# rpng/open_vins

Hardware: NVIDIA H100
Metric: msckf_updates_per_sec (higher is better)
Workload: dtype f64

## Files before the change

open_vins_b200/csrc/k_triangulate.cu:

```cuda
#include "geom.cuh"

__global__ void k_cam_poses(const DevFrame *fr, DevCamPoses *cc) {
  OVB_PDL_ENTER();
  int idx = blockIdx.x * blockDim.x + threadIdx.x;
  int total = fr->n_cams * fr->n_clones;
  if (idx >= total)
    return;
  int cam = idx / fr->n_clones, cl = idx % fr->n_clones;
  dm3 R_ItoC = ld_m3(fr->cam_R[cam]);
  dv3 p_IinC = ld_v3(fr->cam_p[cam]);
  dm3 R_GtoI = ld_m3(fr->clone_R[cl]);
  dv3 p_IinG = ld_v3(fr->clone_p[cl]);
  dm3 R = mul33(R_ItoC, R_GtoI);
  dv3 p = sub3(p_IinG, mTv3(R, p_IinC));
#pragma unroll
  for (int i = 0; i < 9; i++)
    cc->cc_R[cam][cl][i] = R.m[i];
  cc->cc_p[cam][cl][0] = p.x;
  cc->cc_p[cam][cl][1] = p.y;
  cc->cc_p[cam][cl][2] = p.z;
}

void launch_cam_poses(ovb_ctx *ctx) {
  int total = OVB_MAX_CAMS * OVB_MAX_CLONES;
  k_cam_poses<<<(total + 127) / 128, 128, 0, ctx->stream>>>(ctx->d_frame, ctx->d_cc);
}

#define TRI_MAX_WARPS 8
#define TRI_PITCH 33
template <int NV> __device__ __forceinline__ void seq_add(double (&s)[NV], const double (&c)[NV], int count, double *wbuf) {
  const int lane = threadIdx.x & 31;
#pragma unroll
  for (int k = 0; k < NV; k++)
    wbuf[k * TRI_PITCH + lane] = c[k];
  __syncwarp();
  double a = 0.0;
#pragma unroll
  for (int k = 0; k < NV; k++)
    a = (lane == k) ? s[k] : a;
  if (lane < NV) {
    const double *row = wbuf + lane * TRI_PITCH;
    for (int l = 0; l < count; l++)
      a += row[l];
  }
#pragma unroll
  for (int k = 0; k < NV; k++)
    s[k] = __shfl_sync(0xffffffffu, a, k);
  __syncwarp();
}

struct Rel {
  dm3 R;
  dv3 t;
  dv3 q;
};
__device__ __forceinline__ Rel rel_pose(const DevCamPoses *fr, int cam, int cl, const dm3 &R_GtoA, dv3 p_AinG) {
  dm3 Rc = ld_m3(fr->cc_R[cam][cl]);
  dv3 pc = ld_v3(fr->cc_p[cam][cl]);
  Rel r;
  r.R = mul33T(Rc, R_GtoA);
  r.t = mv3(R_GtoA, sub3(pc, p_AinG));
  r.q = negmv3(r.R, r.t);
  return r;
}

__device__ __forceinline__ double lm_cost(const DevCamPoses *fr, const BlobView &bv, int m0, int m1, int lane, const dm3 &R_GtoA, dv3 p_AinG,
                                          double alpha, double beta, double rho, double *wbuf) {
  double err[1] = {0.0};
  for (int base = m0; base < m1; base += 32) {
    const int i = base + lane;
    double c[1] = {0.0};
    if (i < m1) {
      Rel r = rel_pose(fr, bv.cam[i], bv.clone[i], R_GtoA, p_AinG);
      double hi1 = r.R.m[0] * alpha + r.R.m[1] * beta + r.R.m[2] + rho * r.q.x;
      double hi2 = r.R.m[3] * alpha + r.R.m[4] * beta + r.R.m[5] + rho * r.q.y;
      double hi3 = r.R.m[6] * alpha + r.R.m[7] * beta + r.R.m[8] + rho * r.q.z;
      float z0 = (float)(hi1 / hi3), z1 = (float)(hi2 / hi3);
      float r0 = __fsub_rn(bv.uvn[2 * i], z0), r1 = __fsub_rn(bv.uvn[2 * i + 1], z1);
      float nrm = __fsqrt_rn(__fadd_rn(__fmul_rn(r0, r0), __fmul_rn(r1, r1)));
      c[0] = (double)nrm * (double)nrm;
    }
    seq_add<1>(err, c, min(32, m1 - base), wbuf);
  }
  return err[0];
}

__global__ void __launch_bounds__(256) k_triangulate(const DevCamPoses *__restrict__ fr, const DevOpts *__restrict__ dop,
                                                     DevFeat *__restrict__ feats, int n_feats, BlobView bv) {
  OVB_PDL_ENTER();
  __shared__ double tri_stage[TRI_MAX_WARPS][9 * TRI_PITCH];
  double *wbuf = tri_stage[threadIdx.x >> 5];
  int warp = (blockIdx.x * blockDim.x + threadIdx.x) >> 5;
  int lane = threadIdx.x & 31;
  if (warp >= n_feats)
    return;
  DevFeat *F = &feats[warp];
  const ovb_opts &op = dop->o;
  int m0 = F->m0, m1 = F->m1;
  const double qnan = __longlong_as_double(0x7ff8000000000000LL);
  int status = OVB_FEAT_OK;
  dv3 pA = mk3(qnan, qnan, qnan), pG = pA;
  int anchor_cam = -1, anchor_clone = -1;
  if (m1 - m0 < 2) {
    status = OVB_FEAT_FEW_MEAS;
  } else {
    int most = 0;
    anchor_cam = 0;
    for (int k = F->key0; k < F->key1; k++) {
      int key = bv.keys[k];
      int cnt = 0;
      for (int i = m0 + lane; i < m1; i += 32)
        cnt += (bv.cam[i] == key) ? 1 : 0;
#pragma unroll
      for (int o = 16; o > 0; o >>= 1)
        cnt += __shfl_xor_sync(0xffffffffu, cnt, o);
      if (cnt > most) {
        anchor_cam = key;
        most = cnt;
      }
    }
    int ameas = -1;
    for (int i = m0 + lane; i < m1; i += 32)
      if (bv.cam[i] == anchor_cam)
        ameas = i;
#pragma unroll
    for (int o = 16; o > 0; o >>= 1)
      ameas = max(ameas, __shfl_xor_sync(0xffffffffu, ameas, o));
    anchor_clone = bv.clone[ameas];
    dm3 R_GtoA = ld_m3(fr->cc_R[anchor_cam][anchor_clone]);
    dv3 p_AinG = ld_v3(fr->cc_p[anchor_cam][anchor_clone]);
    dv3 p_f;
    if (!op.triangulate_1d) {
      double Ab[9] = {0, 0, 0, 0, 0, 0, 0, 0, 0};
      for (int base = m0; base < m1; base += 32) {
        const int i = base + lane;
        double c[9] = {0, 0, 0, 0, 0, 0, 0, 0, 0};
        if (i < m1) {
          Rel r = rel_pose(fr, bv.cam[i], bv.clone[i], R_GtoA, p_AinG);
          dv3 bi = mTv3(r.R, mk3((double)bv.uvn[2 * i], (double)bv.uvn[2 * i + 1], 1.0));
          double nb = norm3(bi);
          bi = mk3(bi.x / nb, bi.y / nb, bi.z / nb);
          dm3 Bp = skew3(bi);
          dm3 Ai = mulT33(Bp, Bp);
          dv3 Aip = mv3(Ai, r.t);
          c[0] = Ai.m[0], c[1] = Ai.m[1], c[2] = Ai.m[2], c[3] = Ai.m[4], c[4] = Ai.m[5], c[5] = Ai.m[8];
          c[6] = Aip.x, c[7] = Aip.y, c[8] = Aip.z;
        }
        seq_add<9>(Ab, c, min(32, m1 - base), wbuf);
      }
      double A[9] = {Ab[0], Ab[1], Ab[2], Ab[1], Ab[3], Ab[4], Ab[2], Ab[4], Ab[5]};
      double b[3] = {Ab[6], Ab[7], Ab[8]};
      p_f = colpiv_solve3(A, mk3(b[0], b[1], b[2]));
      double condA = cond_sym3(A);
      if (fabs(condA) > op.max_cond_number)
        status = OVB_FEAT_TRI_COND;
      else if (p_f.z < op.min_dist || p_f.z > op.max_dist)
        status = OVB_FEAT_TRI_DEPTH;
      else if (isnan(norm3(p_f)))
        status = OVB_FEAT_TRI_NAN;
    } else {
      dv3 ba = mk3((double)bv.uvn[2 * ameas], (double)bv.uvn[2 * ameas + 1], 1.0);
      double nba = norm3(ba);
      ba = mk3(ba.x / nba, ba.y / nba, ba.z / nba);
      double Ab1[2] = {0.0, 0.0};
      for (int base = m0; base < m1; base += 32) {
        const int i = base + lane;
        double c[2] = {0.0, 0.0};
        if (i < m1 && i != ameas) {
          Rel r = rel_pose(fr, bv.cam[i], bv.clone[i], R_GtoA, p_AinG);
          dv3 bi = mTv3(r.R, mk3((double)bv.uvn[2 * i], (double)bv.uvn[2 * i + 1], 1.0));
          double nb = norm3(bi);
          bi = mk3(bi.x / nb, bi.y / nb, bi.z / nb);
          dm3 Bp = skew3(bi);
          dv3 Bb = mv3(Bp, ba);
          c[0] = dot3(Bb, Bb);
          c[1] = dot3(Bb, mv3(Bp, r.t));
        }
        seq_add<2>(Ab1, c, min(32, m1 - base), wbuf);
      }
      const double A1 = Ab1[0], b1 = Ab1[1];
      double depth = b1 / A1;
      p_f = mk3(depth * ba.x, depth * ba.y, depth * ba.z);
      if (p_f.z < op.min_dist || p_f.z > op.max_dist)
        status = OVB_FEAT_TRI_DEPTH;
      else if (isnan(norm3(p_f)))
        status = OVB_FEAT_TRI_NAN;
    }
    if (status == OVB_FEAT_OK) {
      pA = p_f;
      pG = add3(mTv3(R_GtoA, pA), p_AinG);
    }
    if (status == OVB_FEAT_OK && op.refine_features) {
      double rho = 1 / pA.z;
      double alpha = pA.x / pA.z;
      double beta = pA.y / pA.z;
      double lam = op.init_lamda;
      double eps = 10000;
      int runs = 0;
      bool recompute = true;
      double Hs[6] = {0, 0, 0, 0, 0, 0};
      double g[3] = {0, 0, 0};
      double cost_old = lm_cost(fr, bv, m0, m1, lane, R_GtoA, p_AinG, alpha, beta, rho, wbuf);
      while (runs < op.max_runs && lam < op.max_lamda && eps > op.min_dx) {
        if (recompute) {
#pragma unroll
          for (int k = 0; k < 6; k++)
            Hs[k] = 0.0;
          g[0] = g[1] = g[2] = 0.0;
          double Hg[9] = {0, 0, 0, 0, 0, 0, 0, 0, 0};
          for (int base = m0; base < m1; base += 32) {
            const int i = base + lane;
            double c[9] = {0, 0, 0, 0, 0, 0, 0, 0, 0};
            if (i < m1) {
              Rel r = rel_pose(fr, bv.cam[i], bv.clone[i], R_GtoA, p_AinG);
              double hi1 = r.R.m[0] * alpha + r.R.m[1] * beta + r.R.m[2] + rho * r.q.x;
              double hi2 = r.R.m[3] * alpha + r.R.m[4] * beta + r.R.m[5] + rho * r.q.y;
              double hi3 = r.R.m[6] * alpha + r.R.m[7] * beta + r.R.m[8] + rho * r.q.z;
              double h3sq = hi3 * hi3;
              double H0[3], H1[3];
              H0[0] = (r.R.m[0] * hi3 - hi1 * r.R.m[6]) / h3sq;
              H0[1] = (r.R.m[1] * hi3 - hi1 * r.R.m[7]) / h3sq;
              H0[2] = (r.q.x * hi3 - hi1 * r.q.z) / h3sq;
              H1[0] = (r.R.m[3] * hi3 - hi2 * r.R.m[6]) / h3sq;
              H1[1] = (r.R.m[4] * hi3 - hi2 * r.R.m[7]) / h3sq;
              H1[2] = (r.q.y * hi3 - hi2 * r.q.z) / h3sq;
              float z0 = (float)(hi1 / hi3), z1 = (float)(hi2 / hi3);
              double rd0 = (double)__fsub_rn(bv.uvn[2 * i], z0), rd1 = (double)__fsub_rn(bv.uvn[2 * i + 1], z1);
              c[0] = H0[0] * H0[0] + H1[0] * H1[0];
              c[1] = H0[0] * H0[1] + H1[0] * H1[1];
              c[2] = H0[0] * H0[2] + H1[0] * H1[2];
              c[3] = H0[1] * H0[1] + H1[1] * H1[1];
              c[4] = H0[1] * H0[2] + H1[1] * H1[2];
              c[5] = H0[2] * H0[2] + H1[2] * H1[2];
#pragma unroll
              for (int a = 0; a < 3; a++)
                c[6 + a] = H0[a] * rd0 + H1[a] * rd1;
            }
            seq_add<9>(Hg, c, min(32, m1 - base), wbuf);
          }
#pragma unroll
          for (int k = 0; k < 6; k++)
            Hs[k] = Hg[k];
#pragma unroll
          for (int k = 0; k < 3; k++)
            g[k] = Hg[6 + k];
        }
        double Hl[9] = {Hs[0] * (1.0 + lam), Hs[1], Hs[2], Hs[1], Hs[3] * (1.0 + lam), Hs[4], Hs[2], Hs[4], Hs[5] * (1.0 + lam)};
        dv3 dx = colpiv_solve3(Hl, mk3(g[0], g[1], g[2]));
        double cost = lm_cost(fr, bv, m0, m1, lane, R_GtoA, p_AinG, alpha + dx.x, beta + dx.y, rho + dx.z, wbuf);
        if (cost <= cost_old && (cost_old - cost) / cost_old < op.min_dcost) {
          alpha += dx.x;
          beta += dx.y;
          rho += dx.z;
          eps = 0;
          break;
        }
        if (cost <= cost_old) {
          recompute = true;
          cost_old = cost;
          alpha += dx.x;
          beta += dx.y;
          rho += dx.z;
          runs++;
          lam = lam / op.lam_mult;
          eps = norm3(dx);
        } else {
          recompute = false;
          lam = lam * op.lam_mult;
        }
      }
      pA = mk3(alpha / rho, beta / rho, 1 / rho);
      dv3 q1, q2;
      householder_tangent3(pA, q1, q2);
      double base_line_max = 0.0;
      for (int i = m0 + lane; i < m1; i += 32) {
        dv3 pc = ld_v3(fr->cc_p[bv.cam[i]][bv.clone[i]]);
        dv3 t = mv3(R_GtoA, sub3(pc, p_AinG));
        double a0 = dot3(q1, t), a1 = dot3(q2, t);
        double bl = sqrt(a0 * a0 + a1 * a1);
        if (bl > base_line_max)
          base_line_max = bl;
      }
      base_line_max = warp_max(base_line_max);
      if (pA.z < op.min_dist || pA.z > op.max_dist)
        status = OVB_FEAT_GN_DEPTH;
      else if ((norm3(pA) / base_line_max) > op.max_baseline)
        status = OVB_FEAT_GN_BASELINE;
      else if (isnan(norm3(pA)))
        status = OVB_FEAT_GN_NAN;
      else
        pG = add3(mTv3(R_GtoA, pA), p_AinG);
    }
  }
  if (lane == 0) {
    F->status = status;
    F->anchor_cam = anchor_cam;
    F->anchor_clone = anchor_clone;
    F->p_FinA[0] = pA.x;
    F->p_FinA[1] = pA.y;
    F->p_FinA[2] = pA.z;
    F->p_FinG[0] = pG.x;
    F->p_FinG[1] = pG.y;
    F->p_FinG[2] = pG.z;
    F->chi2 = qnan;
  }
}

void launch_triangulate(ovb_ctx *ctx, int n_feats, BlobView bv) {
  if (n_feats <= 0)
    return;
  int warps_per_cta = (n_feats + ctx->sm_count - 1) / ctx->sm_count;
  warps_per_cta = warps_per_cta < 1 ? 1 : (warps_per_cta > 8 ? 8 : warps_per_cta);
  int grid = (n_feats + warps_per_cta - 1) / warps_per_cta;
  ovb_launch(ctx, k_triangulate, dim3(grid), dim3(warps_per_cta * 32), (size_t)(0), ctx->d_cc, ctx->d_opts, ctx->d_feat, n_feats, bv);
}
```

Before: 2308.

## Assign one CTA per feature with shared-memory pose cache and parallel LM damping candidates

Triangulation now runs one CTA per feature instead of one warp per feature. Relative poses and measurements are cached in dynamic shared memory, so each LM pass reads them there rather than recomputing them from global memory. When a CTA has several warps, each warp evaluates the LM step with a different damping factor and also computes the Hessian at its candidate point, so rejected steps cost fewer serial rounds. The cost is extra syncthreads, more shared memory per block, a host-side occupancy query that picks the warp count, and an optional clock-based probe path behind an ifdef.

```diff
diff --git a/open_vins_b200/csrc/k_triangulate.cu b/open_vins_b200/csrc/k_triangulate.cu
--- a/open_vins_b200/csrc/k_triangulate.cu
+++ b/open_vins_b200/csrc/k_triangulate.cu
@@ -1,4 +1,6 @@
 #include "geom.cuh"
+
+#include <cstdio>
 
 __global__ void k_cam_poses(const DevFrame *fr, DevCamPoses *cc) {
   OVB_PDL_ENTER();
@@ -26,8 +28,13 @@
   k_cam_poses<<<(total + 127) / 128, 128, 0, ctx->stream>>>(ctx->d_frame, ctx->d_cc);
 }
 
-#define TRI_MAX_WARPS 8
+#ifndef TRI_MAX_WARPS
+#define TRI_MAX_WARPS 4
+#endif
 #define TRI_PITCH 33
+#define TRI_NV 10
+#define TRI_CAND 13
+#define TRI_REL 15
 template <int NV> __device__ __forceinline__ void seq_add(double (&s)[NV], const double (&c)[NV], int count, double *wbuf) {
   const int lane = threadIdx.x & 31;
 #pragma unroll
@@ -48,6 +55,11 @@
     s[k] = __shfl_sync(0xffffffffu, a, k);
   __syncwarp();
 }
+
+__host__ __device__ constexpr size_t tri_smem_bytes(int max_meas, int n_warps) {
+  return sizeof(double) * ((size_t)TRI_REL * max_meas + (size_t)n_warps * (TRI_NV * TRI_PITCH + TRI_CAND)) + sizeof(float) * 2 * (size_t)max_meas;
+}
+static_assert(tri_smem_bytes(OVB_MAX_MEAS_PER_FEAT, TRI_MAX_WARPS) <= 227 * 1024, "the longest track must fit one CTA's shared memory");
 
 struct Rel {
   dm3 R;
@@ -63,131 +75,238 @@
   r.q = negmv3(r.R, r.t);
   return r;
 }
-
-__device__ __forceinline__ double lm_cost(const DevCamPoses *fr, const BlobView &bv, int m0, int m1, int lane, const dm3 &R_GtoA, dv3 p_AinG,
-                                          double alpha, double beta, double rho, double *wbuf) {
-  double err[1] = {0.0};
-  for (int base = m0; base < m1; base += 32) {
-    const int i = base + lane;
-    double c[1] = {0.0};
-    if (i < m1) {
-      Rel r = rel_pose(fr, bv.cam[i], bv.clone[i], R_GtoA, p_AinG);
+__device__ __forceinline__ void rel_store(double *rel, int M, int j, const Rel &r) {
+#pragma unroll
+  for (int k = 0; k < 9; k++)
+    rel[k * M + j] = r.R.m[k];
+  rel[9 * M + j] = r.t.x, rel[10 * M + j] = r.t.y, rel[11 * M + j] = r.t.z;
+  rel[12 * M + j] = r.q.x, rel[13 * M + j] = r.q.y, rel[14 * M + j] = r.q.z;
+}
+__device__ __forceinline__ Rel rel_load(const double *rel, int M, int j) {
+  Rel r;
+#pragma unroll
+  for (int k = 0; k < 9; k++)
+    r.R.m[k] = rel[k * M + j];
+  r.t = mk3(rel[9 * M + j], rel[10 * M + j], rel[11 * M + j]);
+  r.q = mk3(rel[12 * M + j], rel[13 * M + j], rel[14 * M + j]);
+  return r;
+}
+
+template <bool HESS>
+__device__ __forceinline__ void lm_pass(const double *rel, const float *uvn, int M, int lane, double alpha, double beta, double rho,
+                                        double (&s)[TRI_NV], double *wbuf) {
+  constexpr int NV = HESS ? TRI_NV : 1;
+  double a[NV];
+#pragma unroll
+  for (int k = 0; k < NV; k++)
+    a[k] = 0.0;
+  for (int base = 0; base < M; base += 32) {
+    const int j = base + lane;
+    double c[NV];
+#pragma unroll
+    for (int k = 0; k < NV; k++)
+      c[k] = 0.0;
+    if (j < M) {
+      const Rel r = rel_load(rel, M, j);
       double hi1 = r.R.m[0] * alpha + r.R.m[1] * beta + r.R.m[2] + rho * r.q.x;
       double hi2 = r.R.m[3] * alpha + r.R.m[4] * beta + r.R.m[5] + rho * r.q.y;
       double hi3 = r.R.m[6] * alpha + r.R.m[7] * beta + r.R.m[8] + rho * r.q.z;
       float z0 = (float)(hi1 / hi3), z1 = (float)(hi2 / hi3);
-      float r0 = __fsub_rn(bv.uvn[2 * i], z0), r1 = __fsub_rn(bv.uvn[2 * i + 1], z1);
+      float r0 = __fsub_rn(uvn[2 * j], z0), r1 = __fsub_rn(uvn[2 * j + 1], z1);
       float nrm = __fsqrt_rn(__fadd_rn(__fmul_rn(r0, r0), __fmul_rn(r1, r1)));
       c[0] = (double)nrm * (double)nrm;
-    }
-    seq_add<1>(err, c, min(32, m1 - base), wbuf);
-  }
-  return err[0];
-}
-
-__global__ void __launch_bounds__(256) k_triangulate(const DevCamPoses *__restrict__ fr, const DevOpts *__restrict__ dop,
-                                                     DevFeat *__restrict__ feats, int n_feats, BlobView bv) {
+      if constexpr (HESS) {
+        double h3sq = hi3 * hi3;
+        double H0[3], H1[3];
+        H0[0] = (r.R.m[0] * hi3 - hi1 * r.R.m[6]) / h3sq;
+        H0[1] = (r.R.m[1] * hi3 - hi1 * r.R.m[7]) / h3sq;
+        H0[2] = (r.q.x * hi3 - hi1 * r.q.z) / h3sq;
+        H1[0] = (r.R.m[3] * hi3 - hi2 * r.R.m[6]) / h3sq;
+        H1[1] = (r.R.m[4] * hi3 - hi2 * r.R.m[7]) / h3sq;
+        H1[2] = (r.q.y * hi3 - hi2 * r.q.z) / h3sq;
+        double rd0 = (double)r0, rd1 = (double)r1;
+        c[1] = H0[0] * H0[0] + H1[0] * H1[0];
+        c[2] = H0[0] * H0[1] + H1[0] * H1[1];
+        c[3] = H0[0] * H0[2] + H1[0] * H1[2];
+        c[4] = H0[1] * H0[1] + H1[1] * H1[1];
+        c[5] = H0[1] * H0[2] + H1[1] * H1[2];
+        c[6] = H0[2] * H0[2] + H1[2] * H1[2];
+#pragma unroll
+        for (int k = 0; k < 3; k++)
+          c[7 + k] = H0[k] * rd0 + H1[k] * rd1;
+      }
+    }
+    seq_add<NV>(a, c, min(32, M - base), wbuf);
+  }
+#pragma unroll
+  for (int k = 0; k < NV; k++)
+    s[k] = a[k];
+}
+
+__global__ void __launch_bounds__(TRI_MAX_WARPS * 32, 16 / TRI_MAX_WARPS) k_triangulate(const DevCamPoses *__restrict__ fr, const DevOpts *__restrict__ dop,
+                                                                    DevFeat *__restrict__ feats, BlobView bv, int max_meas) {
   OVB_PDL_ENTER();
-  __shared__ double tri_stage[TRI_MAX_WARPS][9 * TRI_PITCH];
-  double *wbuf = tri_stage[threadIdx.x >> 5];
-  int warp = (blockIdx.x * blockDim.x + threadIdx.x) >> 5;
-  int lane = threadIdx.x & 31;
-  if (warp >= n_feats)
-    return;
-  DevFeat *F = &feats[warp];
+#ifdef TRI_PROBE
+  const long long t_start = clock64();
+  long long ts[7] = {0, 0, 0, 0, 0, 0, 0};
+#define TRI_STAMP(k) (ts[k] = clock64())
+  __shared__ int s_passes;
+  int n_acc = 0, n_rej = 0, n_rounds = 0;
+  if (threadIdx.x == 0)
+    s_passes = 0;
+#else
+#define TRI_STAMP(k) ((void)0)
+#endif
+  extern __shared__ double tri_smem[];
+  __shared__ int s_anchor[2];
+  __shared__ int s_status;
+  __shared__ double s_pf[3];
+  __shared__ double s_A[9];
+  __shared__ int s_cond_fail;
+  const int nw = blockDim.x >> 5, warp = threadIdx.x >> 5, lane = threadIdx.x & 31;
+  double *rel = tri_smem;
+  double *wbuf = rel + (size_t)TRI_REL * max_meas + warp * (TRI_NV * TRI_PITCH);
+  double *cand = rel + (size_t)TRI_REL * max_meas + nw * (TRI_NV * TRI_PITCH);
+  float *uvn = (float *)(cand + nw * TRI_CAND);
+  DevFeat *F = &feats[blockIdx.x];
   const ovb_opts &op = dop->o;
-  int m0 = F->m0, m1 = F->m1;
+  const int m0 = F->m0, m1 = F->m1, M = m1 - m0;
   const double qnan = __longlong_as_double(0x7ff8000000000000LL);
   int status = OVB_FEAT_OK;
   dv3 pA = mk3(qnan, qnan, qnan), pG = pA;
   int anchor_cam = -1, anchor_clone = -1;
-  if (m1 - m0 < 2) {
+  if (M < 2) {
     status = OVB_FEAT_FEW_MEAS;
   } else {
-    int most = 0;
-    anchor_cam = 0;
-    for (int k = F->key0; k < F->key1; k++) {
-      int key = bv.keys[k];
-      int cnt = 0;
+    if (warp == 0) {
+      int most = 0;
+      int acam = 0;
+      for (int k = F->key0; k < F->key1; k++) {
+        int key = bv.keys[k];
+        int cnt = 0;
+        for (int i = m0 + lane; i < m1; i += 32)
+          cnt += (bv.cam[i] == key) ? 1 : 0;
+#pragma unroll
+        for (int o = 16; o > 0; o >>= 1)
+          cnt += __shfl_xor_sync(0xffffffffu, cnt, o);
+        if (cnt > most) {
+          acam = key;
+          most = cnt;
+        }
+      }
+      int ameas = -1;
       for (int i = m0 + lane; i < m1; i += 32)
-        cnt += (bv.cam[i] == key) ? 1 : 0;
+        if (bv.cam[i] == acam)
+          ameas = i;
 #pragma unroll
       for (int o = 16; o > 0; o >>= 1)
-        cnt += __shfl_xor_sync(0xffffffffu, cnt, o);
-      if (cnt > most) {
-        anchor_cam = key;
-        most = cnt;
-      }
-    }
-    int ameas = -1;
-    for (int i = m0 + lane; i < m1; i += 32)
-      if (bv.cam[i] == anchor_cam)
-        ameas = i;
-#pragma unroll
-    for (int o = 16; o > 0; o >>= 1)
-      ameas = max(ameas, __shfl_xor_sync(0xffffffffu, ameas, o));
+        ameas = max(ameas, __shfl_xor_sync(0xffffffffu, ameas, o));
+      if (lane == 0)
+        s_anchor[0] = acam, s_anchor[1] = ameas;
+    }
+    __syncthreads();
+    TRI_STAMP(0);
+    anchor_cam = s_anchor[0];
+    const int ameas = s_anchor[1];
     anchor_clone = bv.clone[ameas];
     dm3 R_GtoA = ld_m3(fr->cc_R[anchor_cam][anchor_clone]);
     dv3 p_AinG = ld_v3(fr->cc_p[anchor_cam][anchor_clone]);
-    dv3 p_f;
-    if (!op.triangulate_1d) {
-      double Ab[9] = {0, 0, 0, 0, 0, 0, 0, 0, 0};
-      for (int base = m0; base < m1; base += 32) {
-        const int i = base + lane;
-        double c[9] = {0, 0, 0, 0, 0, 0, 0, 0, 0};
-        if (i < m1) {
-          Rel r = rel_pose(fr, bv.cam[i], bv.clone[i], R_GtoA, p_AinG);
-          dv3 bi = mTv3(r.R, mk3((double)bv.uvn[2 * i], (double)bv.uvn[2 * i + 1], 1.0));
-          double nb = norm3(bi);
-          bi = mk3(bi.x / nb, bi.y / nb, bi.z / nb);
-          dm3 Bp = skew3(bi);
-          dm3 Ai = mulT33(Bp, Bp);
-          dv3 Aip = mv3(Ai, r.t);
-          c[0] = Ai.m[0], c[1] = Ai.m[1], c[2] = Ai.m[2], c[3] = Ai.m[4], c[4] = Ai.m[5], c[5] = Ai.m[8];
-          c[6] = Aip.x, c[7] = Aip.y, c[8] = Aip.z;
-        }
-        seq_add<9>(Ab, c, min(32, m1 - base), wbuf);
-      }
-      double A[9] = {Ab[0], Ab[1], Ab[2], Ab[1], Ab[3], Ab[4], Ab[2], Ab[4], Ab[5]};
-      double b[3] = {Ab[6], Ab[7], Ab[8]};
-      p_f = colpiv_solve3(A, mk3(b[0], b[1], b[2]));
-      double condA = cond_sym3(A);
-      if (fabs(condA) > op.max_cond_number)
-        status = OVB_FEAT_TRI_COND;
-      else if (p_f.z < op.min_dist || p_f.z > op.max_dist)
-        status = OVB_FEAT_TRI_DEPTH;
-      else if (isnan(norm3(p_f)))
-        status = OVB_FEAT_TRI_NAN;
-    } else {
-      dv3 ba = mk3((double)bv.uvn[2 * ameas], (double)bv.uvn[2 * ameas + 1], 1.0);
-      double nba = norm3(ba);
-      ba = mk3(ba.x / nba, ba.y / nba, ba.z / nba);
-      double Ab1[2] = {0.0, 0.0};
-      for (int base = m0; base < m1; base += 32) {
-        const int i = base + lane;
-        double c[2] = {0.0, 0.0};
-        if (i < m1 && i != ameas) {
-          Rel r = rel_pose(fr, bv.cam[i], bv.clone[i], R_GtoA, p_AinG);
-          dv3 bi = mTv3(r.R, mk3((double)bv.uvn[2 * i], (double)bv.uvn[2 * i + 1], 1.0));
-          double nb = norm3(bi);
-          bi = mk3(bi.x / nb, bi.y / nb, bi.z / nb);
-          dm3 Bp = skew3(bi);
-          dv3 Bb = mv3(Bp, ba);
-          c[0] = dot3(Bb, Bb);
-          c[1] = dot3(Bb, mv3(Bp, r.t));
-        }
-        seq_add<2>(Ab1, c, min(32, m1 - base), wbuf);
-      }
-      const double A1 = Ab1[0], b1 = Ab1[1];
-      double depth = b1 / A1;
-      p_f = mk3(depth * ba.x, depth * ba.y, depth * ba.z);
-      if (p_f.z < op.min_dist || p_f.z > op.max_dist)
-        status = OVB_FEAT_TRI_DEPTH;
-      else if (isnan(norm3(p_f)))
-        status = OVB_FEAT_TRI_NAN;
-    }
+    for (int j = threadIdx.x; j < M; j += blockDim.x) {
+      rel_store(rel, M, j, rel_pose(fr, bv.cam[m0 + j], bv.clone[m0 + j], R_GtoA, p_AinG));
+      uvn[2 * j] = bv.uvn[2 * (m0 + j)];
+      uvn[2 * j + 1] = bv.uvn[2 * (m0 + j) + 1];
+    }
+    __syncthreads();
+    TRI_STAMP(1);
+    if (warp == 0) {
+      dv3 p_f;
+      if (!op.triangulate_1d) {
+        double Ab[9] = {0, 0, 0, 0, 0, 0, 0, 0, 0};
+        for (int base = 0; base < M; base += 32) {
+          const int j = base + lane;
+          double c[9] = {0, 0, 0, 0, 0, 0, 0, 0, 0};
+          if (j < M) {
+            const Rel r = rel_load(rel, M, j);
+            dv3 bi = mTv3(r.R, mk3((double)uvn[2 * j], (double)uvn[2 * j + 1], 1.0));
+            double nb = norm3(bi);
+            bi = mk3(bi.x / nb, bi.y / nb, bi.z / nb);
+            dm3 Bp = skew3(bi);
+            dm3 Ai = mulT33(Bp, Bp);
+            dv3 Aip = mv3(Ai, r.t);
+            c[0] = Ai.m[0], c[1] = Ai.m[1], c[2] = Ai.m[2], c[3] = Ai.m[4], c[4] = Ai.m[5], c[5] = Ai.m[8];
+            c[6] = Aip.x, c[7] = Aip.y, c[8] = Aip.z;
+          }
+          seq_add<9>(Ab, c, min(32, M - base), wbuf);
+        }
+        double A[9] = {Ab[0], Ab[1], Ab[2], Ab[1], Ab[3], Ab[4], Ab[2], Ab[4], Ab[5]};
+        double b[3] = {Ab[6], Ab[7], Ab[8]};
+        if (lane == 0)
+          for (int k = 0; k < 9; k++)
+            s_A[k] = A[k];
+        p_f = colpiv_solve3(A, mk3(b[0], b[1], b[2]));
+        TRI_STAMP(2);
+        if (nw == 1 && fabs(cond_sym3(A)) > op.max_cond_number)
+          status = OVB_FEAT_TRI_COND;
+        else if (p_f.z < op.min_dist || p_f.z > op.max_dist)
+          status = OVB_FEAT_TRI_DEPTH;
+        else if (isnan(norm3(p_f)))
+          status = OVB_FEAT_TRI_NAN;
+      } else {
+        const int ja = ameas - m0;
+        dv3 ba = mk3((double)uvn[2 * ja], (double)uvn[2 * ja + 1], 1.0);
+        double nba = norm3(ba);
+        ba = mk3(ba.x / nba, ba.y / nba, ba.z / nba);
+        double Ab1[2] = {0.0, 0.0};
+        for (int base = 0; base < M; base += 32) {
+          const int j = base + lane;
+          double c[2] = {0.0, 0.0};
+          if (j < M && j != ja) {
+            const Rel r = rel_load(rel, M, j);
+            dv3 bi = mTv3(r.R, mk3((double)uvn[2 * j], (double)uvn[2 * j + 1], 1.0));
+            double nb = norm3(bi);
+            bi = mk3(bi.x / nb, bi.y / nb, bi.z / nb);
+            dm3 Bp = skew3(bi);
+            dv3 Bb = mv3(Bp, ba);
+            c[0] = dot3(Bb, Bb);
+            c[1] = dot3(Bb, mv3(Bp, r.t));
+          }
+          seq_add<2>(Ab1, c, min(32, M - base), wbuf);
+        }
+        const double A1 = Ab1[0], b1 = Ab1[1];
+        double depth = b1 / A1;
+        p_f = mk3(depth * ba.x, depth * ba.y, depth * ba.z);
+        if (p_f.z < op.min_dist || p_f.z > op.max_dist)
+          status = OVB_FEAT_TRI_DEPTH;
+        else if (isnan(norm3(p_f)))
+          status = OVB_FEAT_TRI_NAN;
+      }
+      if (lane == 0) {
+        s_status = status;
+        s_pf[0] = p_f.x, s_pf[1] = p_f.y, s_pf[2] = p_f.z;
+      }
+    }
+    __syncthreads();
+    TRI_STAMP(3);
+    status = s_status;
+    const bool refine = status == OVB_FEAT_OK && op.refine_features;
+    double s[TRI_NV] = {0, 0, 0, 0, 0, 0, 0, 0, 0, 0};
+    if (warp == 0 && refine) {
+      lm_pass<true>(rel, uvn, M, lane, s_pf[0] / s_pf[2], s_pf[1] / s_pf[2], 1 / s_pf[2], s, wbuf);
+      if (lane == 0)
+        for (int k = 0; k < TRI_NV; k++)
+          cand[k] = s[k];
+    }
+    if (nw > 1 && warp == nw - 1 && !op.triangulate_1d) {
+      const bool fail = fabs(cond_sym3(s_A)) > op.max_cond_number;
+      if (lane == 0)
+        s_cond_fail = fail;
+    }
+    __syncthreads();
+    TRI_STAMP(4);
+    if (nw > 1 && !op.triangulate_1d && s_cond_fail)
+      status = OVB_FEAT_TRI_COND;
     if (status == OVB_FEAT_OK) {
-      pA = p_f;
+      pA = mk3(s_pf[0], s_pf[1], s_pf[2]);
       pG = add3(mTv3(R_GtoA, pA), p_AinG);
     }
     if (status == OVB_FEAT_OK && op.refine_features) {
@@ -197,102 +316,126 @@
       double lam = op.init_lamda;
       double eps = 10000;
       int runs = 0;
-      bool recompute = true;
-      double Hs[6] = {0, 0, 0, 0, 0, 0};
-      double g[3] = {0, 0, 0};
-      double cost_old = lm_cost(fr, bv, m0, m1, lane, R_GtoA, p_AinG, alpha, beta, rho, wbuf);
-      while (runs < op.max_runs && lam < op.max_lamda && eps > op.min_dx) {
+#ifdef TRI_PROBE
+      if (threadIdx.x == 0)
+        s_passes++;
+#endif
+      double cost_old = cand[0];
+      double Hs[6] = {cand[1], cand[2], cand[3], cand[4], cand[5], cand[6]};
+      double g[3] = {cand[7], cand[8], cand[9]};
+      TRI_STAMP(5);
+      __syncthreads();
+      bool done = false, recompute = false;
+      while (!done && runs < op.max_runs && lam < op.max_lamda && eps > op.min_dx) {
         if (recompute) {
+          lm_pass<true>(rel, uvn, M, lane, alpha, beta, rho, s, wbuf);
 #pragma unroll
           for (int k = 0; k < 6; k++)
-            Hs[k] = 0.0;
-          g[0] = g[1] = g[2] = 0.0;
-          double Hg[9] = {0, 0, 0, 0, 0, 0, 0, 0, 0};
-          for (int base = m0; base < m1; base += 32) {
-            const int i = base + lane;
-            double c[9] = {0, 0, 0, 0, 0, 0, 0, 0, 0};
-            if (i < m1) {
-              Rel r = rel_pose(fr, bv.cam[i], bv.clone[i], R_GtoA, p_AinG);
-              double hi1 = r.R.m[0] * alpha + r.R.m[1] * beta + r.R.m[2] + rho * r.q.x;
-              double hi2 = r.R.m[3] * alpha + r.R.m[4] * beta + r.R.m[5] + rho * r.q.y;
-              double hi3 = r.R.m[6] * alpha + r.R.m[7] * beta + r.R.m[8] + rho * r.q.z;
-              double h3sq = hi3 * hi3;
-              double H0[3], H1[3];
-              H0[0] = (r.R.m[0] * hi3 - hi1 * r.R.m[6]) / h3sq;
-              H0[1] = (r.R.m[1] * hi3 - hi1 * r.R.m[7]) / h3sq;
-              H0[2] = (r.q.x * hi3 - hi1 * r.q.z) / h3sq;
-              H1[0] = (r.R.m[3] * hi3 - hi2 * r.R.m[6]) / h3sq;
-              H1[1] = (r.R.m[4] * hi3 - hi2 * r.R.m[7]) / h3sq;
-              H1[2] = (r.q.y * hi3 - hi2 * r.q.z) / h3sq;
-              float z0 = (float)(hi1 / hi3), z1 = (float)(hi2 / hi3);
-              double rd0 = (double)__fsub_rn(bv.uvn[2 * i], z0), rd1 = (double)__fsub_rn(bv.uvn[2 * i + 1], z1);
-              c[0] = H0[0] * H0[0] + H1[0] * H1[0];
-              c[1] = H0[0] * H0[1] + H1[0] * H1[1];
-              c[2] = H0[0] * H0[2] + H1[0] * H1[2];
-              c[3] = H0[1] * H0[1] + H1[1] * H1[1];
-              c[4] = H0[1] * H0[2] + H1[1] * H1[2];
-              c[5] = H0[2] * H0[2] + H1[2] * H1[2];
-#pragma unroll
-              for (int a = 0; a < 3; a++)
-                c[6 + a] = H0[a] * rd0 + H1[a] * rd1;
+            Hs[k] = s[1 + k];
+#pragma unroll
+          for (int k = 0; k < 3; k++)
+            g[k] = s[7 + k];
+          recompute = false;
+#ifdef TRI_PROBE
+          if (lane == 0)
+            atomicAdd(&s_passes, 1);
+#endif
+        }
+        double lw = lam;
+        for (int w = 0; w < warp; w++)
+          lw = lw * op.lam_mult;
+        if (lw < op.max_lamda) {
+          double Hl[9] = {Hs[0] * (1.0 + lw), Hs[1], Hs[2], Hs[1], Hs[3] * (1.0 + lw), Hs[4], Hs[2], Hs[4], Hs[5] * (1.0 + lw)};
+          dv3 dx = colpiv_solve3(Hl, mk3(g[0], g[1], g[2]));
+          if (nw > 1)
+            lm_pass<true>(rel, uvn, M, lane, alpha + dx.x, beta + dx.y, rho + dx.z, s, wbuf);
+          else
+            lm_pass<false>(rel, uvn, M, lane, alpha + dx.x, beta + dx.y, rho + dx.z, s, wbuf);
+          if (lane == 0) {
+            double *c = cand + warp * TRI_CAND;
+            for (int k = 0; k < TRI_NV; k++)
+              c[k] = s[k];
+            c[TRI_NV] = dx.x, c[TRI_NV + 1] = dx.y, c[TRI_NV + 2] = dx.z;
+#ifdef TRI_PROBE
+            atomicAdd(&s_passes, 1);
+#endif
+          }
+        }
+        __syncthreads();
+#ifdef TRI_PROBE
+        n_rounds++;
+#endif
+        for (int w = 0; w < nw && runs < op.max_runs && lam < op.max_lamda && eps > op.min_dx; w++) {
+          const double *c = cand + w * TRI_CAND;
+          const double cost = c[0];
+          const dv3 dx = mk3(c[TRI_NV], c[TRI_NV + 1], c[TRI_NV + 2]);
+          if (cost <= cost_old && (cost_old - cost) / cost_old < op.min_dcost) {
+            alpha += dx.x;
+            beta += dx.y;
+            rho += dx.z;
+            eps = 0;
+            done = true;
+#ifdef TRI_PROBE
+            n_acc++;
+#endif
+            break;
+          }
+          if (cost <= cost_old) {
+            cost_old = cost;
+            alpha += dx.x;
+            beta += dx.y;
+            rho += dx.z;
+            runs++;
+            lam = lam / op.lam_mult;
+            eps = norm3(dx);
+            if (nw > 1) {
+#pragma unroll
+              for (int k = 0; k < 6; k++)
+                Hs[k] = c[1 + k];
+#pragma unroll
+              for (int k = 0; k < 3; k++)
+                g[k] = c[7 + k];
+            } else {
+              recompute = true;
             }
-            seq_add<9>(Hg, c, min(32, m1 - base), wbuf);
+#ifdef TRI_PROBE
+            n_acc++;
+#endif
+            break;
           }
-#pragma unroll
-          for (int k = 0; k < 6; k++)
-            Hs[k] = Hg[k];
-#pragma unroll
-          for (int k = 0; k < 3; k++)
-            g[k] = Hg[6 + k];
-        }
-        double Hl[9] = {Hs[0] * (1.0 + lam), Hs[1], Hs[2], Hs[1], Hs[3] * (1.0 + lam), Hs[4], Hs[2], Hs[4], Hs[5] * (1.0 + lam)};
-        dv3 dx = colpiv_solve3(Hl, mk3(g[0], g[1], g[2]));
-        double cost = lm_cost(fr, bv, m0, m1, lane, R_GtoA, p_AinG, alpha + dx.x, beta + dx.y, rho + dx.z, wbuf);
-        if (cost <= cost_old && (cost_old - cost) / cost_old < op.min_dcost) {
-          alpha += dx.x;
-          beta += dx.y;
-          rho += dx.z;
-          eps = 0;
-          break;
-        }
-        if (cost <= cost_old) {
-          recompute = true;
-          cost_old = cost;
-          alpha += dx.x;
-          beta += dx.y;
-          rho += dx.z;
-          runs++;
-          lam = lam / op.lam_mult;
-          eps = norm3(dx);
-        } else {
-          recompute = false;
           lam = lam * op.lam_mult;
-        }
-      }
+#ifdef TRI_PROBE
+          n_rej++;
+#endif
+        }
+        __syncthreads();
+      }
+      TRI_STAMP(6);
       pA = mk3(alpha / rho, beta / rho, 1 / rho);
-      dv3 q1, q2;
-      householder_tangent3(pA, q1, q2);
-      double base_line_max = 0.0;
-      for (int i = m0 + lane; i < m1; i += 32) {
-        dv3 pc = ld_v3(fr->cc_p[bv.cam[i]][bv.clone[i]]);
-        dv3 t = mv3(R_GtoA, sub3(pc, p_AinG));
-        double a0 = dot3(q1, t), a1 = dot3(q2, t);
-        double bl = sqrt(a0 * a0 + a1 * a1);
-        if (bl > base_line_max)
-          base_line_max = bl;
-      }
-      base_line_max = warp_max(base_line_max);
-      if (pA.z < op.min_dist || pA.z > op.max_dist)
-        status = OVB_FEAT_GN_DEPTH;
-      else if ((norm3(pA) / base_line_max) > op.max_baseline)
-        status = OVB_FEAT_GN_BASELINE;
-      else if (isnan(norm3(pA)))
-        status = OVB_FEAT_GN_NAN;
-      else
-        pG = add3(mTv3(R_GtoA, pA), p_AinG);
-    }
-  }
-  if (lane == 0) {
+      if (warp == 0) {
+        dv3 q1, q2;
+        householder_tangent3(pA, q1, q2);
+        double base_line_max = 0.0;
+        for (int j = lane; j < M; j += 32) {
+          dv3 t = mk3(rel[9 * M + j], rel[10 * M + j], rel[11 * M + j]);
+          double a0 = dot3(q1, t), a1 = dot3(q2, t);
+          double bl = sqrt(a0 * a0 + a1 * a1);
+          if (bl > base_line_max)
+            base_line_max = bl;
+        }
+        base_line_max = warp_max(base_line_max);
+        if (pA.z < op.min_dist || pA.z > op.max_dist)
+          status = OVB_FEAT_GN_DEPTH;
+        else if ((norm3(pA) / base_line_max) > op.max_baseline)
+          status = OVB_FEAT_GN_BASELINE;
+        else if (isnan(norm3(pA)))
+          status = OVB_FEAT_GN_NAN;
+        else
+          pG = add3(mTv3(R_GtoA, pA), p_AinG);
+      }
+    }
+  }
+  if (threadIdx.x == 0) {
     F->status = status;
     F->anchor_cam = anchor_cam;
     F->anchor_clone = anchor_clone;
@@ -303,14 +446,28 @@
     F->p_FinG[1] = pG.y;
     F->p_FinG[2] = pG.z;
     F->chi2 = qnan;
+#ifdef TRI_PROBE
+    printf("TRI_PROBE f=%d M=%d warps=%d passes=%d accepted=%d rejected=%d rounds=%d cycles=%lld ph=%lld,%lld,%lld,%lld,%lld,%lld,%lld\n", blockIdx.x, M, nw, M < 2 ? 0 : s_passes,
+           n_acc, n_rej, n_rounds, clock64() - t_start, ts[0] - t_start, ts[1] - t_start, ts[2] - t_start, ts[3] - t_start, ts[4] - t_start, ts[5] - t_start, ts[6] - t_start);
+#endif
   }
 }
 
 void launch_triangulate(ovb_ctx *ctx, int n_feats, BlobView bv) {
   if (n_feats <= 0)
     return;
-  int warps_per_cta = (n_feats + ctx->sm_count - 1) / ctx->sm_count;
-  warps_per_cta = warps_per_cta < 1 ? 1 : (warps_per_cta > 8 ? 8 : warps_per_cta);
-  int grid = (n_feats + warps_per_cta - 1) / warps_per_cta;
-  ovb_launch(ctx, k_triangulate, dim3(grid), dim3(warps_per_cta * 32), (size_t)(0), ctx->d_cc, ctx->d_opts, ctx->d_feat, n_feats, bv);
-}
+  if (!ctx->attr_done[5]) {
+    cudaFuncSetAttribute(k_triangulate, cudaFuncAttributeMaxDynamicSharedMemorySize, (int)tri_smem_bytes(OVB_MAX_MEAS_PER_FEAT, TRI_MAX_WARPS));
+    ctx->attr_done[5] = 1;
+  }
+  const DevFeat &longest = ctx->h_feat[ctx->h_feat[0].sched];
+  const int max_meas = longest.m1 - longest.m0 < 2 ? 2 : longest.m1 - longest.m0;
+  int nw = TRI_MAX_WARPS;
+  for (; nw > 1; nw >>= 1) {
+    int per_sm = 0;
+    cudaOccupancyMaxActiveBlocksPerMultiprocessor(&per_sm, k_triangulate, nw * 32, tri_smem_bytes(max_meas, nw));
+    if ((long long)per_sm * ctx->sm_count >= n_feats)
+      break;
+  }
+  ovb_launch(ctx, k_triangulate, dim3(n_feats), dim3(nw * 32), tri_smem_bytes(max_meas, nw), ctx->d_cc, ctx->d_opts, ctx->d_feat, bv, max_meas);
+}
```

Result: faster. 2373 (median of 6 runs) (+2.8%).
